# Ipsedo/MARLClassification

Measured on NVIDIA B200. Metric: image_episodes_per_sec, higher is better.
Workload: dtype tf32x3

## Files before the change

marlclassification_b200/csrc/engine.cu:

```cuda
#include <stdarg.h>
#include <string.h>

#include <algorithm>

#include <string>
#include <vector>

#include <nvtx3/nvToolsExt.h>

#include "../../include/marlc.h"
#include "kernels.cuh"
#include "chain.cuh"
#include "tc.cuh"

namespace marlc {

int g_launch_count = 0;
long g_simt_gemm_launches = 0, g_tc_gemm_launches = 0;
static thread_local char g_err[512] = "";
void set_error(const char* fmt, ...) {
    va_list ap;
    va_start(ap, fmt);
    vsnprintf(g_err, sizeof(g_err), fmt, ap);
    va_end(ap);
}
thread_local int g_pdl = 0, g_pdl_trig = 0;
bool pdl_enabled() {
    static const bool on = !(getenv("MARLC_PDL") && atoi(getenv("MARLC_PDL")) == 0);
    return on;
}
int pdl_edge(int bit) {
    static const int mask = getenv("MARLC_PDL_MASK") ? atoi(getenv("MARLC_PDL_MASK")) : 125;
    return (mask & bit) ? 1 : 0;
}
int pdl_trig_mode(int bwd) {
    static const int t = getenv("MARLC_PDL_TRIG") ? atoi(getenv("MARLC_PDL_TRIG")) : 1;
    return (t >> (bwd ? 1 : 0)) & 1;
}
int pdl_trigger_early() { return g_pdl_trig; }

struct ParamInfo {
    std::string name;
    int64_t offset;
    int ndim;
    int64_t shape[4];
    int64_t numel;
};
struct BufInfo {
    std::string name;
    size_t offset, bytes;
};

}

using namespace marlc;

struct NvtxRange {
    explicit NvtxRange(const char* name) { nvtxRangePushA(name); }
    ~NvtxRange() { nvtxRangePop(); }
};

struct marlc_engine {
    marlc_config cfg;
    int M, TM, F, Kin, L;
    CnnDesc cnn;
    int cnn_sz[MAX_CNN_LAYERS];
    std::vector<ParamInfo> params;
    int64_t param_floats = 0;
    std::vector<BufInfo> bufs;
    size_t ws_bytes = 0;
    char* ws = nullptr;
    float* P = nullptr;
    float* G = nullptr;
    int last_launches = 0;
    int debug_stop = 0;
    cudaStream_t side[2] = {nullptr, nullptr};
    cudaStream_t hp = nullptr;
    int bwd_chunks = 1;
    cudaEvent_t ev[64];
    int n_ev = 0, ev_i = 0;
    cudaEvent_t next_event() { cudaEvent_t x = ev[ev_i]; ev_i = (ev_i + 1) % n_ev; return x; }
    int chain(cudaStream_t from, cudaStream_t to) {
        cudaEvent_t x = next_event();
        MARLC_CUDA(cudaEventRecord(x, from));
        MARLC_CUDA(cudaStreamWaitEvent(to, x, 0));
        return 0;
    }

    void add_param(const std::string& name, std::initializer_list<int64_t> shape) {
        ParamInfo p;
        p.name = "_ModelsWrapper__" + name;
        p.ndim = (int)shape.size();
        p.numel = 1;
        int i = 0;
        for (int k = 0; k < 4; ++k) p.shape[k] = 1;
        for (auto s : shape) { p.shape[i++] = s; p.numel *= s; }
        p.offset = param_floats;
        param_floats += (p.numel + 63) / 64 * 64;
        params.push_back(p);
    }
    void add_buf(const std::string& name, size_t bytes) {
        BufInfo b{name, ws_bytes, bytes};
        ws_bytes += (bytes + 255) / 256 * 256;
        bufs.push_back(b);
    }
    const ParamInfo* find_param(const std::string& suffix) const {
        for (auto& p : params)
            if (p.name == "_ModelsWrapper__" + suffix) return &p;
        return nullptr;
    }
    float* prm(const std::string& suffix) const { return P + find_param(suffix)->offset; }
    bool lo_on = false;
    bool h_lo_ok = false;
    const float* lo_of(const float* p) const {
        if (!lo_on || !p) return nullptr;
        struct R { const float* base; size_t n; const float* lo; };
        const size_t Ms = (size_t)M, T1 = (size_t)cfg.T + 1;
        const R r[] = {{P, (size_t)param_floats, buf("params_lo")},
                       {buf("H"), T1 * Ms * cfg.n_b, buf("H_lo")},
                       {buf("Hc"), T1 * Ms * cfg.n_a, buf("Hc_lo")}
                       };
        for (int i = 0; i < 3; ++i) {
            const R& q = r[i];
            if (i > 0 && !h_lo_ok) break;
            if (q.lo && p >= q.base && p < q.base + q.n) return q.lo + (p - q.base);
        }
        return nullptr;
    }
    TcOperand op(const float* p, long ld, bool mn = false) const {
        TcOperand o = tc_op(p, ld, mn);
        o.lo = lo_of(p);
        return o;
    }
    float* grd(const std::string& suffix) const { return G + find_param(suffix)->offset; }
    template <typename T = float>
    T* buf(const std::string& name) const {
        for (auto& b : bufs)
            if (b.name == name) return reinterpret_cast<T*>(ws + b.offset);
        return nullptr;
    }
};

static const char* CNN_PREFIX = "map_obs._Generic2dCnnModule__layers.";
static const char* LSTM_B = "belief_unit._LSTMCellWrapper__lstm.";
static const char* LSTM_A = "action_unit._LSTMCellWrapper__lstm.";

static void add_block(marlc_engine* e, const std::string& name, int i, int n_in, int n_out, bool norm) {
    e->add_param(name + "." + std::to_string(i) + ".weight", {n_out, n_in});
    e->add_param(name + "." + std::to_string(i) + ".bias", {n_out});
    if (norm) {
        e->add_param(name + "." + std::to_string(i + 1) + ".weight", {n_out});
        e->add_param(name + "." + std::to_string(i + 1) + ".bias", {n_out});
    }
}

extern "C" int marlc_version(void) { return 1; }

extern "C" long marlc_selftest_fastdiv(int d_max, int stride) {
    long bad = 0;
    if (stride < 1) stride = 1;
    for (int d = 1; d <= d_max; ++d) {
// ... 75 lines not shown

    const size_t M = e->M, TM = e->TM, T = c->T, F4 = sizeof(float);
    e->add_buf("rng_state", 2 * sizeof(uint64_t));
    e->add_buf("pos_hist", (T + 1) * M * 2 * sizeof(int));
    e->add_buf("npos", (T + 1) * M * 2 * F4);
    e->add_buf("act", TM * sizeof(int));
    e->add_buf("zero_act", M * sizeof(int64_t));
    e->add_buf("step_pos", TM * 2 * sizeof(int64_t));
    for (int l = 0; l < e->L; ++l) e->add_buf("cnn_y" + std::to_string(l), TM * e->cnn_sz[l] * F4);
    e->add_buf("U", TM * e->Kin * F4);
    e->add_buf("msg", (T + 1) * M * c->n_m * F4);
    e->add_buf("coll", TM * c->n_m * F4);
    e->add_buf("dec_y1", TM * 2 * c->n_m * F4);
    e->add_buf("dec_s1", TM * 2 * c->n_m * F4);
    e->add_buf("dec_y2", TM * c->n_m_o * F4);
    e->add_buf("pos_y", TM * c->n_d * F4);
    e->add_buf("H", (T + 1) * M * c->n_b * F4);
    e->add_buf("Cb", (T + 1) * M * c->n_b * F4);
    e->add_buf("Hc", (T + 1) * M * c->n_a * F4);
    e->add_buf("Cc", (T + 1) * M * c->n_a * F4);
    e->add_buf("gates_b", TM * 4 * c->n_b * F4);
    e->add_buf("gates_a", TM * 4 * c->n_a * F4);
    e->add_buf("enc_y1", TM * 2 * c->n_m * F4);
    e->add_buf("enc_s1", TM * 2 * c->n_m * F4);
    e->add_buf("enc_y2", TM * c->n_m * F4);
    e->add_buf("pol_y1", TM * c->nl_a * F4);
    e->add_buf("pol_s1", TM * c->nl_a * F4);
    e->add_buf("probs", TM * c->n_actions * F4);
    e->add_buf("cri_y1", TM * c->nl_a * F4);
    e->add_buf("cri_s1", TM * c->nl_a * F4);
    e->add_buf("prd_y1", TM * c->nl_b * F4);
    e->add_buf("prd_s1", TM * c->nl_b * F4);
    e->add_buf("step_preds", TM * c->nb_class * F4);
    e->add_buf("step_log_probas", TM * F4);
    e->add_buf("step_values", TM * F4);
    e->add_buf("rewards", TM * F4);
    e->add_buf("returns", TM * F4);
    e->add_buf("adv", TM * F4);
    e->add_buf("loss_stats", 16 * sizeof(double));
    e->add_buf("loss_out", 8 * F4);
    e->add_buf("d_preds", TM * c->nb_class * F4);
    e->add_buf("d_logp", TM * F4);
    e->add_buf("d_values", TM * F4);
    const size_t nl_max = (size_t)std::max(c->nl_a, c->nl_b);
    e->add_buf("d_pol_logits", TM * c->n_actions * F4);
    e->add_buf("scratchS", TM * nl_max * F4);
    e->add_buf("scratchY", TM * nl_max * F4);
    e->add_buf("scratchS2", TM * nl_max * F4);
    e->add_buf("scratchY2", TM * nl_max * F4);
    e->add_buf("scratchS3", TM * nl_max * F4);
    e->add_buf("scratchY3", TM * nl_max * F4);
    e->add_buf("dH_heads", TM * c->n_b * F4);
    e->add_buf("dHc_heads", TM * c->n_a * F4);
    e->add_buf("dgates_b", TM * 4 * c->n_b * F4);
    e->add_buf("dgates_a", TM * 4 * c->n_a * F4);
    e->add_buf("dU", TM * e->Kin * F4);
    e->add_buf("d_enc_y2", TM * c->n_m * F4);
    e->add_buf("d_enc_y1", TM * 2 * c->n_m * F4);
    e->add_buf("d_dec_y2", TM * c->n_m_o * F4);
    e->add_buf("d_dec_y1", TM * 2 * c->n_m * F4);
    e->add_buf("d_pos_y", TM * c->n_d * F4);
    e->add_buf("tmpS", M * 2 * c->n_m * F4);
    e->add_buf("dcoll", M * c->n_m * F4);
    e->add_buf("dmsg", M * c->n_m * F4);
    e->add_buf("dh_hist", TM * c->n_b * F4);
    e->add_buf("dhc_hist", TM * c->n_a * F4);
    e->add_buf("dh", M * c->n_b * F4);
    e->add_buf("dc0", M * c->n_b * F4);
    e->add_buf("dc1", M * c->n_b * F4);
    e->add_buf("dhc", M * c->n_a * F4);
    e->add_buf("dcc0", M * c->n_a * F4);
    e->add_buf("dcc1", M * c->n_a * F4);
    if (e->cfg.use_chains)
        for (int l = 0; l < e->L; ++l)
            e->add_buf("cnn_wT" + std::to_string(l), (size_t)d.cout[l] * d.cin[l] * 9 * F4);
    if (e->lo_on) {
        e->add_buf("params_lo", (size_t)e->param_floats * F4);
        e->add_buf("U_lo", M * e->Kin * F4);
        e->add_buf("H_lo", (T + 1) * M * c->n_b * F4);
        e->add_buf("Hc_lo", (T + 1) * M * c->n_a * F4);
        e->add_buf("dgates_b_lo", M * 4 * c->n_b * F4);
        e->add_buf("dgates_a_lo", M * 4 * c->n_a * F4);
    }
    for (int l = 0; l < e->L; ++l) {
        const size_t npos = (size_t)d.hout[l] * d.hout[l];
        e->add_buf("cnn_dY" + std::to_string(l), TM * npos * d.cout[l] * F4);
        e->add_buf("cnn_col" + std::to_string(l), TM * npos * (size_t)((d.cin[l] * 9 + 3) & ~3) * F4);
        e->add_buf("cnn_gnpart" + std::to_string(l), TM * 2 * d.cout[l] * F4);
        if (l > 0) e->add_buf("cnn_dcol" + std::to_string(l), TM * npos * d.cin[l] * 9 * F4);
    }
    *out = e;
    return 0;
}

extern "C" void marlc_engine_destroy(marlc_engine* e) {
    if (!e) return;
    for (int i = 0; i < e->n_ev; ++i) cudaEventDestroy(e->ev[i]);
    for (int i = 0; i < 2; ++i)
        if (e->side[i]) cudaStreamDestroy(e->side[i]);
    if (e->hp) cudaStreamDestroy(e->hp);
    delete e;
}
extern "C" int marlc_engine_param_count(const marlc_engine* e) { return (int)e->params.size(); }
extern "C" int64_t marlc_engine_param_floats(const marlc_engine* e) { return e->param_floats; }
extern "C" int marlc_engine_param_info(const marlc_engine* e, int idx, char* name, int64_t* offset, int* ndim,
                                       int64_t* shape) {
    MARLC_CHECK(idx >= 0 && idx < (int)e->params.size(), "param index %d out of range", idx);
    const ParamInfo& p = e->params[idx];
    strncpy(name, p.name.c_str(), 127);
    name[127] = 0;
    *offset = p.offset;
    *ndim = p.ndim;
    for (int k = 0; k < 4; ++k) shape[k] = p.shape[k];
    return 0;
}
extern "C" size_t marlc_engine_workspace_bytes(const marlc_engine* e) { return e->ws_bytes; }
extern "C" int marlc_engine_buffer(const marlc_engine* e, const char* name, size_t* offset, size_t* nbytes) {
    for (auto& b : e->bufs)
        if (b.name == name) {
            *offset = b.offset;
            *nbytes = b.bytes;
            return 0;
        }
    MARLC_FAIL("unknown workspace buffer '%s'", name);
}

extern "C" int marlc_engine_bind(marlc_engine* e, void* workspace, float* params, float* grads) {
    MARLC_CHECK(workspace && params, "bind: null workspace / params");
    MARLC_CHECK(((uintptr_t)workspace & 255) == 0 && ((uintptr_t)params & 255) == 0, "bind: buffers must be 256-byte aligned");
    e->ws = (char*)workspace;
    e->P = params;
    e->G = grads;
    if (e->n_ev == 0) {
        for (int i = 0; i < 2; ++i) MARLC_CUDA(cudaStreamCreateWithFlags(&e->side[i], cudaStreamNonBlocking));
        int least = 0, greatest = 0;
        MARLC_CUDA(cudaDeviceGetStreamPriorityRange(&least, &greatest));
        MARLC_CUDA(cudaStreamCreateWithPriority(&e->hp, cudaStreamNonBlocking, greatest));
        if (const char* env = getenv("MARLC_BWD_CHUNKS")) e->bwd_chunks = std::max(1, atoi(env));
        for (int i = 0; i < 64; ++i) {
            MARLC_CUDA(cudaEventCreateWithFlags(&e->ev[i], cudaEventDisableTiming));
            e->n_ev = i + 1;
        }
    }
    for (int l = 0; l < e->L; ++l) {
        e->cnn.w[l] = e->prm(CNN_PREFIX + std::to_string(3 * l) + ".weight");
        e->cnn.b[l] = e->prm(CNN_PREFIX + std::to_string(3 * l) + ".bias");
        e->cnn.gn_w[l] = e->prm(CNN_PREFIX + std::to_string(3 * l + 1) + ".weight");
        e->cnn.gn_b[l] = e->prm(CNN_PREFIX + std::to_string(3 * l + 1) + ".bias");
        e->cnn.wT[l] = e->cfg.use_chains ? e->buf("cnn_wT" + std::to_string(l)) : nullptr;
    }
    return 0;
}

__global__ void seed_kernel(uint64_t* st, uint64_t seed) { st[0] = seed; st[1] = 0; }
extern "C" int marlc_engine_seed(marlc_engine* e, uint64_t seed, void* stream) {
    MARLC_CHECK(e->ws, "engine not bound");
    seed_kernel<<<1, 1, 0, (cudaStream_t)stream>>>(e->buf<uint64_t>("rng_state"), seed);
    MARLC_LAUNCH_CHECK();
    return 0;
}


static inline TcOperand tc_op_lo(const float* p, const float* lo, long ld) {
    TcOperand o = tc_op(p, ld);
    o.lo = lo;
    return o;
}
struct SplitLoArgs { const float* src[3]; float* dst[3]; long n[3]; };
__global__ void __launch_bounds__(256) split_lo_kernel(const SplitLoArgs a) {
    const int k = blockIdx.y;
    const long n4 = a.n[k] >> 2;
    const float4* s4 = reinterpret_cast<const float4*>(a.src[k]);
// ... 491 lines not shown
            TcGemmArgs a;
            a.A = tc_op(Yp, c.nl_a); a.B = e->op(e->prm("policy.0.weight"), c.n_a, true); a.K = c.nl_a;
            a.A2 = tc_op(Yc, c.nl_a); a.B2 = e->op(e->prm("critic.0.weight"), c.n_a, true); a.K2 = c.nl_a;
            a.C = e->buf("dHc_heads"); a.ldc = c.n_a; a.M = TM; a.N = c.n_a; a.x3 = x3_of(e); a.allow_split = 1;
            if (tc_operand_ok(a.A) && tc_operand_ok(a.B) && tc_operand_ok(a.A2) && tc_operand_ok(a.B2)) {
                MARLC_TRY(tc_gemm(a, s));
                dual = true;
            }
        }
        if (!dual) {
            MARLC_TRY(G_nn(e, Yp, c.nl_a, e->prm("policy.0.weight"), c.n_a, e->buf("dHc_heads"), c.n_a, TM, c.nl_a, c.n_a, 0, s));
            MARLC_TRY(G_nn(e, Yc, c.nl_a, e->prm("critic.0.weight"), c.n_a, e->buf("dHc_heads"), c.n_a, TM, c.nl_a, c.n_a, 1, s));
        }
        MARLC_TRY(e->chain(sp, s));
        MARLC_TRY(head_bwd_params(e, "predict", e->buf("d_preds"), c.nb_class, e->buf("prd_s1"), Yq,
                                  H + (size_t)M * c.n_b, c.n_b, c.nl_b, sp));
        MARLC_TRY(e->chain(s, sc));
        MARLC_TRY(head_bwd_params(e, "policy", e->buf("d_pol_logits"), c.n_actions, e->buf("pol_s1"), Yp,
                                  Hc + (size_t)M * c.n_a, c.n_a, c.nl_a, sc));
        MARLC_TRY(head_bwd_params(e, "critic", e->buf("d_values"), 1, e->buf("cri_s1"), Yc, Hc + (size_t)M * c.n_a,
                                  c.n_a, c.nl_a, sc));
    } else {
        MARLC_TRY(head_bwd(e, "predict", e->buf("d_preds"), c.nb_class, e->buf("prd_s1"), e->buf("prd_y1"),
                           H + (size_t)M * c.n_b, c.n_b, c.nl_b, e->buf("dH_heads"), 0, s, 1));
        MARLC_TRY(policy_logit_grad(e->buf("d_logp"), e->buf("probs"), e->buf<int>("act"), e->buf("d_pol_logits"), TM,
                                    c.n_actions, s));
        MARLC_TRY(head_bwd(e, "policy", e->buf("d_pol_logits"), c.n_actions, e->buf("pol_s1"), e->buf("pol_y1"),
                           Hc + (size_t)M * c.n_a, c.n_a, c.nl_a, e->buf("dHc_heads"), 0, s));
        MARLC_TRY(head_bwd(e, "critic", e->buf("d_values"), 1, e->buf("cri_s1"), e->buf("cri_y1"), Hc + (size_t)M * c.n_a,
                           c.n_a, c.nl_a, e->buf("dHc_heads"), 1, s));
    }

    }
    auto join_sides = [&]() -> int {
        if (!c.use_chains) return 0;
        MARLC_TRY(e->chain(e->side[0], s));
        MARLC_TRY(e->chain(e->side[1], s));
        return 0;
    };
    if (e->debug_stop == 1) { MARLC_TRY(join_sides()); e->last_launches = g_launch_count - start; return 0; }
    const bool par = c.use_chains != 0;
    auto batched = [&](int t0, int t1, cudaStream_t sL, cudaStream_t s1, cudaStream_t s0) -> int {
        NvtxRange nvtx_batched("marlc/backward/batched_grads");
        const size_t r0 = (size_t)t0 * M;
        const int R = (t1 - t0) * M;
        if (R <= 0) return 0;
        {
            const float* dgb = e->buf("dgates_b") + r0 * 4 * c.n_b;
            const float* dga = e->buf("dgates_a") + r0 * 4 * c.n_a;
            const float* Ur = e->buf("U") + r0 * Kin;
            const std::string pb = LSTM_B, pa = LSTM_A;
            const TnProblem ih[2] = {{dgb, 4L * c.n_b, Ur, Kin, e->grd(pb + "weight_ih"), Kin, R, 4 * c.n_b, Kin},
                                     {dga, 4L * c.n_a, Ur, Kin, e->grd(pa + "weight_ih"), Kin, R, 4 * c.n_a, Kin}};
            const TnProblem hh[2] = {{dgb, 4L * c.n_b, H + r0 * c.n_b, c.n_b, e->grd(pb + "weight_hh"), c.n_b, R, 4 * c.n_b, c.n_b},
                                     {dga, 4L * c.n_a, Hc + r0 * c.n_a, c.n_a, e->grd(pa + "weight_hh"), c.n_a, R, 4 * c.n_a, c.n_a}};
            MARLC_TRY(G_tn_group(e, ih, 2, sL));
            MARLC_TRY(G_tn_group(e, hh, 2, sL));
            MARLC_TRY(colsum_add2(dgb, 4 * c.n_b, e->grd(pb + "bias_ih"), e->grd(pb + "bias_hh"), R, 4 * c.n_b, sL));
            MARLC_TRY(colsum_add2(dga, 4 * c.n_a, e->grd(pa + "bias_ih"), e->grd(pa + "bias_hh"), R, 4 * c.n_a, sL));
        }
        {
            const int Re = (std::min(t1, T - 1) - t0) * M;
            const TnProblem enc[2] = {
                {e->buf("d_enc_y2") + r0 * c.n_m, c.n_m, e->buf("enc_s1") + r0 * 2 * c.n_m, 2L * c.n_m,
                 e->grd("encode_msg.3.weight"), 2L * c.n_m, Re, c.n_m, 2 * c.n_m},
                {e->buf("d_enc_y1") + r0 * 2 * c.n_m, 2L * c.n_m, H + (r0 + M) * c.n_b, c.n_b,
                 e->grd("encode_msg.0.weight"), c.n_b, Re, 2 * c.n_m, c.n_b}};
            if (Re > 0) MARLC_TRY(G_tn_group(e, enc, 2, s1));
            const TnProblem dec[2] = {
                {e->buf("d_dec_y2") + r0 * c.n_m_o, c.n_m_o, e->buf("dec_s1") + r0 * 2 * c.n_m, 2L * c.n_m,
                 e->grd("decode_msg.3.weight"), 2L * c.n_m, R, c.n_m_o, 2 * c.n_m},
                {e->buf("d_dec_y1") + r0 * 2 * c.n_m, 2L * c.n_m, e->buf("coll") + r0 * c.n_m, c.n_m,
                 e->grd("decode_msg.0.weight"), c.n_m, R, 2 * c.n_m, c.n_m}};
            MARLC_TRY(G_tn_group(e, dec, 2, s1));
        }
        MARLC_TRY(block_bwd_norm(e, "map_pos", 0, dU + r0 * Kin + F + c.n_m_o, Kin, e->buf("pos_y") + r0 * c.n_d, R, c.n_d,
                                 e->buf("d_pos_y") + r0 * c.n_d, s1));
        MARLC_TRY(G_tn(e, e->buf("d_pos_y") + r0 * c.n_d, c.n_d, e->buf("npos") + r0 * 2, 2, e->grd("map_pos.0.weight"), 2,
                       R, c.n_d, 2, s1));
        const CnnDesc& d = e->cnn;
        const float* ysave[MAX_CNN_LAYERS];
        CnnBwdBuffers bb;
        float* dcol[MAX_CNN_LAYERS] = {nullptr};
        for (int l = 0; l < e->L; ++l) {
            const size_t npos = (size_t)d.hout[l] * d.hout[l];
            ysave[l] = e->buf("cnn_y" + std::to_string(l)) + (par ? r0 * e->cnn_sz[l] : 0);
            bb.dY[l] = e->buf("cnn_dY" + std::to_string(l)) + (par ? r0 * npos * d.cout[l] : 0);
            bb.col[l] = e->buf("cnn_col" + std::to_string(l)) + (par ? r0 * npos * (size_t)((d.cin[l] * 9 + 3) & ~3) : 0);
            bb.gnpart[l] = e->buf("cnn_gnpart" + std::to_string(l)) + (par ? r0 * 2 * d.cout[l] : 0);
            if (l > 0) dcol[l] = e->buf("cnn_dcol" + std::to_string(l)) + (par ? r0 * npos * d.cin[l] * 9 : 0);
        }
        auto conv_weight_grad = [&](int l, cudaStream_t st) -> int {
            const int npos = d.hout[l] * d.hout[l], kk = d.cin[l] * 9, co = d.cout[l];
            const int pitch = (par && l == 0) ? (kk + 3) & ~3 : kk;
            return G_tn(e, bb.dY[l], co, bb.col[l], pitch, e->grd(CNN_PREFIX + std::to_string(3 * l) + ".weight"), kk,
                        R * npos, co, kk, st);
        };
        if (!par) {
            MARLC_TRY(cnn_bwd(e->cnn, img, e->buf<int>("pos_hist"), c.nb, c.H, c.W, M, 0, TM, ysave, dU, Kin, bb, s0));
            for (int l = 0; l < e->L; ++l) {
                const int npos = d.hout[l] * d.hout[l], co = d.cout[l];
                const std::string cw = CNN_PREFIX + std::to_string(3 * l), gn = CNN_PREFIX + std::to_string(3 * l + 1);
                MARLC_TRY(conv_weight_grad(l, s0));
                MARLC_TRY(colsum_add(bb.dY[l], co, e->grd(cw + ".bias"), R * npos, co, s0));
                MARLC_TRY(colsum_add(bb.gnpart[l], 2 * co, e->grd(gn + ".weight"), R, co, s0));
                MARLC_TRY(colsum_add(bb.gnpart[l] + co, 2 * co, e->grd(gn + ".bias"), R, co, s0));
            }
            return 0;
        }
        MARLC_TRY(cnn_im2col_input(img, e->buf<int>("pos_hist") + r0 * 2, bb.col[0], R, M, c.nb, c.C, d.cin[0], c.H, c.W,
                                   c.f, d.hout[0], s1));
        for (int l = e->L - 1; l >= 0; --l) {
            CnnBwdLayerArgs la;
            memset(&la, 0, sizeof(la));
            la.cout = d.cout[l]; la.ho = d.hout[l]; la.groups = d.groups[l]; la.P = R;
            la.Y = ysave[l]; la.gn_w = d.gn_w[l]; la.gn_b = d.gn_b[l];
            const bool top = (l == e->L - 1);
            la.dOut = top ? dU + r0 * Kin : nullptr; la.lddo = Kin;
            la.dColNext = top ? nullptr : dcol[l + 1];
            la.ho_next = top ? 1 : d.hout[l + 1];
            la.dY = bb.dY[l]; la.gnpart = nullptr;
            la.d_gn_w = e->grd(CNN_PREFIX + std::to_string(3 * l + 1) + ".weight");
            la.d_gn_b = e->grd(CNN_PREFIX + std::to_string(3 * l + 1) + ".bias");
            la.d_conv_b = e->grd(CNN_PREFIX + std::to_string(3 * l) + ".bias");
            la.colNext = top ? nullptr : bb.col[l + 1];
            MARLC_TRY(cnn_bwd_layer(la, s0));
            if (l > 0) {
                const int npos = d.hout[l] * d.hout[l], kk = d.cin[l] * 9;
                MARLC_TRY(G_nn_on(e, bb.dY[l], d.cout[l], d.w[l], kk, dcol[l], kk, R * npos, d.cout[l], kk, s0));
            }
        }
        {
            cudaStream_t fan[3] = {s0, s1, sL};
            cudaEvent_t done = e->next_event();
            MARLC_CUDA(cudaEventRecord(done, s0));
            if (s1 != s0) MARLC_CUDA(cudaStreamWaitEvent(s1, done, 0));
            if (sL != s0) MARLC_CUDA(cudaStreamWaitEvent(sL, done, 0));
            for (int l = e->L - 1, i = 0; l >= 0; --l, ++i) MARLC_TRY(conv_weight_grad(l, l == 0 ? s1 : fan[(i & 1) ? 2 : 0]));
        }
        return 0;
    };
    NvtxRange nvtx_sweep("marlc/backward/sweep");
    float* dh = e->buf("dh");
    float* dhc = e->buf("dhc");
    float* dc[2] = {e->buf("dc0"), e->buf("dc1")};
    float* dcc[2] = {e->buf("dcc0"), e->buf("dcc1")};
    float* dmsg = e->buf("dmsg");
    float* tmpS = e->buf("tmpS");
    MARLC_CUDA(cudaMemsetAsync(dh, 0, sizeof(float) * (size_t)M * c.n_b, s));
    MARLC_CUDA(cudaMemsetAsync(dhc, 0, sizeof(float) * (size_t)M * c.n_a, s));
    MARLC_CUDA(cudaMemsetAsync(dc[0], 0, sizeof(float) * (size_t)M * c.n_b, s));
    MARLC_CUDA(cudaMemsetAsync(dcc[0], 0, sizeof(float) * (size_t)M * c.n_a, s));
    int cur = 0;
    static const int unfused_min_m = getenv("MARLC_SWEEP_UNFUSED_MIN_M") ? atoi(getenv("MARLC_SWEEP_UNFUSED_MIN_M")) : 4096;
    const bool chain_sweep = c.use_chains && M < unfused_min_m;
    if (chain_sweep) {
        float* dcoll = e->buf("dcoll");
        float* dh_hist = e->buf("dh_hist");
        float* dhc_hist = e->buf("dhc_hist");
        MARLC_CUDA(cudaMemsetAsync(dU, 0, sizeof(float) * (size_t)TM * Kin, s));
        MARLC_CUDA(cudaMemsetAsync(dh_hist, 0, sizeof(float) * (size_t)TM * c.n_b, s));
        MARLC_CUDA(cudaMemsetAsync(dhc_hist, 0, sizeof(float) * (size_t)TM * c.n_a, s));
        const bool profiling_stop = e->debug_stop == 2 || e->debug_stop == 21 || e->debug_stop == 22;
        const int nch = profiling_stop ? 0 : std::max(1, std::min(e->bwd_chunks, T));
        cudaStream_t sw = e->hp, s0 = e->side[0], s1 = e->side[1];
        MARLC_TRY(e->chain(s, sw));
        int chunk_hi = T, next_chunk = nch - 1;
        for (int t = T - 1; t >= 0; --t) {
            float* dgb = e->buf("dgates_b") + (size_t)t * M * 4 * c.n_b;
            float* dga = e->buf("dgates_a") + (size_t)t * M * 4 * c.n_a;
            float* dgb_lo = e->lo_on ? e->buf("dgates_b_lo") : nullptr;
            float* dga_lo = e->lo_on ? e->buf("dgates_a_lo") : nullptr;
            BwdPreArgs bp;
            memset(&bp, 0, sizeof(bp));
            bp.dcoll = (t < T - 1) ? dcoll : nullptr;
            bp.e0 = chain_lin(e, "encode_msg", 0, c.n_b, 2 * c.n_m, true);
            bp.e3 = chain_lin(e, "encode_msg", 3, 2 * c.n_m, c.n_m, true);
            bp.enc_y1 = e->buf("enc_y1") + (size_t)t * M * 2 * c.n_m;
            bp.enc_y2 = e->buf("enc_y2") + (size_t)t * M * c.n_m;
            bp.d_enc_y1 = e->buf("d_enc_y1") + (size_t)t * M * 2 * c.n_m;
            bp.d_enc_y2 = e->buf("d_enc_y2") + (size_t)t * M * c.n_m;
            bp.dh_carry[0] = (t < T - 1) ? dh_hist + (size_t)(t + 1) * M * c.n_b : nullptr;
            bp.dh_carry[1] = (t < T - 1) ? dhc_hist + (size_t)(t + 1) * M * c.n_a : nullptr;
            bp.dh_heads[0] = e->buf("dH_heads") + (size_t)t * M * c.n_b;
            bp.dh_heads[1] = e->buf("dHc_heads") + (size_t)t * M * c.n_a;
            bp.dc_next[0] = (t < T - 1) ? dc[cur] : nullptr;
            bp.dc_next[1] = (t < T - 1) ? dcc[cur] : nullptr;
            bp.gates[0] = e->buf("gates_b") + (size_t)t * M * 4 * c.n_b;
            bp.gates[1] = e->buf("gates_a") + (size_t)t * M * 4 * c.n_a;
            bp.c_prev[0] = Cb + (size_t)t * M * c.n_b;
            bp.c_prev[1] = Cc + (size_t)t * M * c.n_a;
            bp.c_new[0] = Cb + (size_t)(t + 1) * M * c.n_b;
            bp.c_new[1] = Cc + (size_t)(t + 1) * M * c.n_a;
            bp.dgates[0] = dgb; bp.dgates[1] = dga;
            bp.dgates_lo[0] = dgb_lo; bp.dgates_lo[1] = dga_lo;
            bp.dc_prev[0] = dc[cur ^ 1]; bp.dc_prev[1] = dcc[cur ^ 1];
            bp.n[0] = c.n_b; bp.n[1] = c.n_a;
            bp.Na = c.na; bp.Nb = c.nb; bp.M = M; bp.n_m = c.n_m;
            {
                PdlScope pdl(t < T - 1 && pdl_edge(PDL_BWD_PRE), pdl_trig_mode(1));
                MARLC_TRY(bwd_pre(bp, sw));
            }
            cur ^= 1;
            if (e->debug_stop == 21) continue;
            float* dUt = dU + (size_t)t * M * Kin;
            float* dh_t = dh_hist + (size_t)t * M * c.n_b;
            float* dhc_t = dhc_hist + (size_t)t * M * c.n_a;
            bool tc_dx = false;
            if (c.use_tc && c.n_a >= 16 && c.n_b >= 16) {
                TcGemmArgs g[3];
                g[0].A = tc_op_lo(dgb, dgb_lo, 4 * c.n_b); g[0].B = e->op(e->prm(std::string(LSTM_B) + "weight_ih"), Kin, true); g[0].K = 4 * c.n_b;
                g[0].A2 = tc_op_lo(dga, dga_lo, 4 * c.n_a); g[0].B2 = e->op(e->prm(std::string(LSTM_A) + "weight_ih"), Kin, true); g[0].K2 = 4 * c.n_a;
                g[0].C = dUt; g[0].ldc = Kin; g[0].M = M; g[0].N = Kin;
// ... 285 lines not shown
```

marlclassification_b200/csrc/kernels.cuh:

```cuda
#pragma once
#include "common.cuh"

namespace marlc {

int patch_gather_i64(const float* img, const int64_t* pos, float* obs, int Na, int B, int C, int H, int W, int f,
                     cudaStream_t s);
int patch_gather_i32(const float* img, const int* pos, float* obs, int Na, int B, int C, int H, int W, int f,
                     cudaStream_t s);
int transition_i64(int64_t* pos, const int64_t* act, const int64_t* table, int nA, int M, int f, int H, int W,
                   float* npos, int* err, cudaStream_t s);
int normalized_positions_i64(const int64_t* pos, float* out, int M, int H, int W, cudaStream_t s);

struct EpisodeInitArgs {
    const int64_t* pos0;
    const float* hidden0[4];
    const uint64_t* rng_state;
    int* pos;
    float* npos;
    float* hidden[4];
    float* msg0;
    int width[4];
    int M, n_m, H, W, f;
};
int episode_init(const EpisodeInitArgs& a, cudaStream_t s);
int rng_advance(uint64_t* rng_state, cudaStream_t s);

struct PolicyActArgs {
    const float* s1;
    const float* W3;
    const float* b3;
    const int64_t* act_in;
    const uint64_t* rng_state;
    const int* pos_in;
    float* probs;
    float* logp;
    int* act_out;
    int* pos_out;
    int64_t* step_pos;
    float* npos_out;
    int moves[32];
    int M, nl, nA, t, f, H, W;
};
int policy_act(const PolicyActArgs& a, cudaStream_t s);

constexpr int MAX_CNN_LAYERS = 6;
struct CnnDesc {
    int L;
    int cin[MAX_CNN_LAYERS], cout[MAX_CNN_LAYERS], groups[MAX_CNN_LAYERS];
    int hin[MAX_CNN_LAYERS], hout[MAX_CNN_LAYERS];
    int f;
    int img_c;
    int out_size;
    const float* w[MAX_CNN_LAYERS];
    const float* b[MAX_CNN_LAYERS];
    const float* gn_w[MAX_CNN_LAYERS];
    const float* gn_b[MAX_CNN_LAYERS];
    const float* wT[MAX_CNN_LAYERS];
};
int cnn_fwd(const CnnDesc& d, const float* img, const int* pos, const float* patch, int B, int H, int W, int M,
            float* const* y_save, float* out, long ldo, cudaStream_t s);

struct CnnBwdBuffers {
    float* dY[MAX_CNN_LAYERS];
    float* col[MAX_CNN_LAYERS];
    float* gnpart[MAX_CNN_LAYERS];
};
int cnn_bwd(const CnnDesc& d, const float* img, const int* pos_hist, int B, int H, int W, int M, int p0, int P,
            const float* const* y_save, const float* dOut, long lddo, const CnnBwdBuffers& buf, cudaStream_t s);

int cnn_weights_transpose(const CnnDesc& d, float* const* wT, cudaStream_t s);

struct CnnBwdLayerArgs {
    int cout, ho, groups;
    int P;
    const float* Y;
    const float* gn_w;
    const float* gn_b;
    const float* dOut;
    long lddo;
    const float* dColNext;
    int ho_next;
    float* dY;
    float* gnpart;
    float* d_gn_w;
    float* d_gn_b;
    float* d_conv_b;
    float* colNext;
};
int cnn_bwd_layer(const CnnBwdLayerArgs& a, cudaStream_t s);
int cnn_im2col_input(const float* img, const int* pos_hist, float* col, int P, int M, int B, int img_c, int cin, int H,
                     int W, int f, int ho, cudaStream_t s);

struct LossArgs {
    const float* preds;
    const float* logp;
    const float* values;
    const int64_t* targets;
    float* rewards;
    float* returns;
    float* adv;
    double* stats;
    float* d_preds;
    float* d_logp;
    float* d_values;
    float* loss_out;
    int T, Na, Nb, Nc;
    float gamma;
};
int loss_phase_a(const LossArgs& a, cudaStream_t s);
int loss_phase_b(const LossArgs& a, cudaStream_t s);
int policy_logit_grad(const float* d_logp, const float* probs, const int* act, float* dlogits, int R, int nA,
                      cudaStream_t s);

}
```

Measured before the change: 19870.

## Fuse backward of first two CNN layers into one persistent kernel

Adds a persistent kernel that fuses, for the first two conv layers, the input-gradient GEMM, col2im, GroupNorm+SiLU backward, and the weight, bias and norm gradient reductions. Per-patch tiles are staged into shared memory with double-buffered cp.async, and gradients are accumulated in registers and flushed with atomics. This removes the im2col/dcol/gnpart workspace buffers and several launches and global round-trips. The trade-off is a fixed-shape specialisation, plain FP32 math instead of tensor cores for these layers, and atomic accumulation that makes gradient sums order-dependent.

```diff
diff --git a/marlclassification_b200/csrc/cnn_bwd_fused.cu b/marlclassification_b200/csrc/cnn_bwd_fused.cu
--- /dev/null
+++ b/marlclassification_b200/csrc/cnn_bwd_fused.cu
@@ -0,0 +1,300 @@
+#include <algorithm>
+
+#include "common.cuh"
+#include "kernels.cuh"
+
+namespace marlc {
+
+namespace {
+constexpr float GN_EPS1 = 1e-5f;
+constexpr int CI = 3, C0 = 16, C1 = 32, H0 = 6, H1 = 3, FW = 12;
+constexpr int N0 = H0 * H0, N1 = H1 * H1, T0 = C0 * N0, K1 = C0 * 9, K0 = CI * 9;
+constexpr int NW = 8;
+constexpr int THREADS = NW * 32;
+constexpr int ACT_LD = N0 + 1;
+constexpr int S_DY1 = N1 * C1;
+constexpr int S_X = T0;
+constexpr int S_IMG = CI * FW * FW;
+constexpr int S_IN = S_DY1 + S_X + S_IMG;
+constexpr int S_DZ = T0;
+constexpr int S_ACT = C0 * ACT_LD;
+constexpr int S_DCOL = N1 * K1;
+constexpr int S_WIN = 2 * S_IN + S_DZ + S_ACT + S_DCOL;
+constexpr int S_TOTAL = C1 * K1 + NW * S_WIN + 3 * C0;
+static_assert(THREADS / 2 == (C1 / 4) * C0, "dW1 ownership: two halves of (4 output x 1 input channel) blocks");
+static_assert(C0 % 4 == 0 && K1 <= 5 * 32 && (S_DY1 % 4) == 0 && (T0 % 4) == 0 && (S_IN % 4) == 0 && (S_WIN % 4) == 0, "layout");
+__device__ __forceinline__ void cp_async16(float* dst, const float* src) {
+    asm volatile("cp.async.cg.shared.global [%0], [%1], 16;" ::"r"((unsigned)__cvta_generic_to_shared(dst)), "l"(src)
+                 : "memory");
+}
+__device__ __forceinline__ void cp_async4(float* dst, const float* src) {
+    asm volatile("cp.async.ca.shared.global [%0], [%1], 4;" ::"r"((unsigned)__cvta_generic_to_shared(dst)), "l"(src)
+                 : "memory");
+}
+}
+
+struct CnnBwdFused10Args {
+    int P, M, B, img_c, H, W;
+    const float* img;
+    const int* pos_hist;
+    const float* dY1;
+    const float* Y0;
+    const float* w1;
+    const float* gn_w0;
+    const float* gn_b0;
+    int groups0;
+    float* dW1;
+    float* dW0;
+    float* d_gn_w0;
+    float* d_gn_b0;
+    float* d_conv_b0;
+};
+
+__global__ void __launch_bounds__(THREADS, 1) cnn_bwd_fused10_kernel(const CnnBwdFused10Args a) {
+    extern __shared__ __align__(16) float sm[];
+    float* sW1 = sm;
+    float* win0 = sm + C1 * K1;
+    float* cta_acc = win0 + NW * S_WIN;
+    const int tid = threadIdx.x, lane = tid & 31, warp = tid >> 5;
+    for (int i = tid; i < C1 * K1 / 4; i += THREADS) reinterpret_cast<float4*>(sW1)[i] = __ldg(reinterpret_cast<const float4*>(a.w1) + i);
+    for (int i = tid; i < 3 * C0; i += THREADS) cta_acc[i] = 0.f;
+
+    float* w_in = win0 + warp * S_WIN;
+    float* w_dz = w_in + 2 * S_IN;
+    float* w_act = w_dz + S_DZ;
+    float* w_dcol = w_act + S_ACT;
+
+    const int h1 = tid >> 7, cq1 = (tid & 127) >> 4, ci1 = tid & 15;
+    const bool own0 = tid < 12 * (N0 / 2);
+    const int cb0 = tid % 12, cq0 = cb0 / 3, ci0 = cb0 % 3, s0 = tid / 12;
+    float acc1[4][9], acc0[4][9];
+#pragma unroll
+    for (int c = 0; c < 4; ++c)
+#pragma unroll
+        for (int k = 0; k < 9; ++k) acc1[c][k] = acc0[c][k] = 0.f;
+    __syncthreads();
+
+    const int G = a.groups0, cpg = C0 / G, ng = cpg * N0;
+    const float inv = 1.0f / (float)ng;
+    const int ntiles = (a.P + NW - 1) / NW;
+    auto issue = [&](int tile, int buf) {
+        if (tile >= ntiles) return;
+        const int p = tile * NW + warp;
+        float* dy1 = w_in + buf * S_IN;
+        float* x = dy1 + S_DY1;
+        float* im = x + S_X;
+        if (p < a.P) {
+            const float* g1 = a.dY1 + (long)p * S_DY1;
+            for (int i = lane; i < S_DY1 / 4; i += 32) cp_async16(dy1 + 4 * i, g1 + 4 * i);
+            const float* g0 = a.Y0 + (long)p * T0;
+            for (int i = lane; i < T0 / 4; i += 32) cp_async16(x + 4 * i, g0 + 4 * i);
+            const int b = (p % a.M) % a.B, py = __ldg(a.pos_hist + 2 * (long)p), px = __ldg(a.pos_hist + 2 * (long)p + 1);
+            const float* src = a.img + ((long)b * a.img_c * a.H + py) * a.W + px;
+            for (int e = lane; e < S_IMG; e += 32) {
+                const int c = e / (FW * FW), r = e - c * FW * FW, y = r / FW, xx = r - y * FW;
+                cp_async4(im + e, src + ((long)c * a.H + y) * a.W + xx);
+            }
+        } else {
+            for (int i = lane; i < S_IN; i += 32) dy1[i] = 0.f;
+        }
+    };
+    issue(blockIdx.x, 0);
+    asm volatile("cp.async.commit_group;" ::: "memory");
+    int cur = 0;
+    for (int tile = blockIdx.x; tile < ntiles; tile += gridDim.x, cur ^= 1) {
+        issue(tile + gridDim.x, cur ^ 1);
+        asm volatile("cp.async.commit_group;" ::: "memory");
+        asm volatile("cp.async.wait_group 1;" ::: "memory");
+        __syncwarp();
+        float* w_dy1 = w_in + cur * S_IN;
+        float* w_x = w_dy1 + S_DY1;
+        {
+            float acc[N1][5];
+#pragma unroll
+            for (int o = 0; o < N1; ++o)
+#pragma unroll
+                for (int q = 0; q < 5; ++q) acc[o][q] = 0.f;
+            const bool q4 = lane + 128 < K1;
+#pragma unroll 4
+            for (int co = 0; co < C1; ++co) {
+                float wv[5];
+#pragma unroll
+                for (int q = 0; q < 4; ++q) wv[q] = sW1[co * K1 + lane + 32 * q];
+                wv[4] = q4 ? sW1[co * K1 + lane + 128] : 0.f;
+#pragma unroll
+                for (int o = 0; o < N1; ++o) {
+                    const float d = w_dy1[o * C1 + co];
+#pragma unroll
+                    for (int q = 0; q < 5; ++q) acc[o][q] = fmaf(d, wv[q], acc[o][q]);
+                }
+            }
+#pragma unroll
+            for (int o = 0; o < N1; ++o) {
+#pragma unroll
+                for (int q = 0; q < 4; ++q) w_dcol[o * K1 + lane + 32 * q] = acc[o][q];
+                if (q4) w_dcol[o * K1 + lane + 128] = acc[o][4];
+            }
+        }
+        __syncwarp();
+        for (int e = lane; e < T0; e += 32) {
+            const int c = e / N0, pos = e - c * N0, iy = pos / H0, ix = pos - iy * H0;
+            float acc = 0.f;
+#pragma unroll
+            for (int ky = 0; ky < 3; ++ky) {
+                const int ty = iy + 1 - ky;
+                if (ty < 0 || (ty & 1) || (ty >> 1) >= H1) continue;
+#pragma unroll
+                for (int kx = 0; kx < 3; ++kx) {
+                    const int tx = ix + 1 - kx;
+                    if (tx < 0 || (tx & 1) || (tx >> 1) >= H1) continue;
+                    acc += w_dcol[((ty >> 1) * H1 + (tx >> 1)) * K1 + c * 9 + ky * 3 + kx];
+                }
+            }
+            w_dz[e] = acc;
+        }
+        __syncwarp();
+        for (int g = 0; g < G; ++g) {
+            float* xg = w_x + g * ng;
+            float* dg = w_dz + g * ng;
+            float s = 0.f;
+            for (int e = lane; e < ng; e += 32) s += xg[e];
+            const float mean = warp_sum(s) * inv;
+            float v = 0.f;
+            for (int e = lane; e < ng; e += 32) { const float d = xg[e] - mean; v += d * d; }
+            const float rstd = 1.0f / sqrtf(warp_sum(v) * inv + GN_EPS1);
+            float s1 = 0.f, s2 = 0.f;
+            for (int e = lane; e < ng; e += 32) {
+                const int cl = e / N0, c = g * cpg + cl;
+                const float gam = __ldg(a.gn_w0 + c);
+                const float x = (xg[e] - mean) * rstd, z = x * gam + __ldg(a.gn_b0 + c);
+                const float sg = sigmoidf_(z);
+                w_act[c * ACT_LD + (e - cl * N0)] = z * sg;
+                const float d = dg[e] * (sg * (1.f + z * (1.f - sg)));
+                xg[e] = x;
+                dg[e] = d;
+                s1 += d * gam;
+                s2 += d * gam * x;
+            }
+            s1 = warp_sum(s1) * inv;
+            s2 = warp_sum(s2) * inv;
+            __syncwarp();
+            for (int cc = lane; cc < cpg; cc += 32) {
+                float t1 = 0.f, t2 = 0.f;
+                for (int q = 0; q < N0; ++q) { const float d = dg[cc * N0 + q]; t1 += d * xg[cc * N0 + q]; t2 += d; }
+                atomicAdd(&cta_acc[g * cpg + cc], t1);
+                atomicAdd(&cta_acc[C0 + g * cpg + cc], t2);
+            }
+            __syncwarp();
+            for (int e = lane; e < ng; e += 32) {
+                const int c = g * cpg + e / N0;
+                dg[e] = rstd * (dg[e] * __ldg(a.gn_w0 + c) - s1 - xg[e] * s2);
+            }
+            __syncwarp();
+            for (int cc = lane; cc < cpg; cc += 32) {
+                float t3 = 0.f;
+                for (int q = 0; q < N0; ++q) t3 += dg[cc * N0 + q];
+                atomicAdd(&cta_acc[2 * C0 + g * cpg + cc], t3);
+            }
+        }
+        __syncthreads();
+#pragma unroll 1
+        for (int w = h1; w < NW; w += 2) {
+            const float* dy = win0 + w * S_WIN + cur * S_IN;
+            const float* act = win0 + w * S_WIN + 2 * S_IN + S_DZ + ci1 * ACT_LD;
+#pragma unroll
+            for (int o = 0; o < N1; ++o) {
+                const int oy = o / H1, ox = o - oy * H1;
+                const float4 d = *reinterpret_cast<const float4*>(dy + o * C1 + 4 * cq1);
+#pragma unroll
+                for (int ky = 0; ky < 3; ++ky) {
+                    const int iy = 2 * oy - 1 + ky;
+#pragma unroll
+                    for (int kx = 0; kx < 3; ++kx) {
+                        const int ix = 2 * ox - 1 + kx;
+                        if (iy < 0 || ix < 0) continue;
+                        const float v = act[iy * H0 + ix];
+                        acc1[0][ky * 3 + kx] = fmaf(d.x, v, acc1[0][ky * 3 + kx]);
+                        acc1[1][ky * 3 + kx] = fmaf(d.y, v, acc1[1][ky * 3 + kx]);
+                        acc1[2][ky * 3 + kx] = fmaf(d.z, v, acc1[2][ky * 3 + kx]);
+                        acc1[3][ky * 3 + kx] = fmaf(d.w, v, acc1[3][ky * 3 + kx]);
+                    }
+                }
+            }
+        }
+        if (own0) {
+#pragma unroll 1
+            for (int w = 0; w < NW; ++w) {
+                const float* dz = win0 + w * S_WIN + 2 * S_IN + 4 * cq0 * N0;
+                const float* im = win0 + w * S_WIN + cur * S_IN + S_DY1 + S_X + ci0 * FW * FW;
+#pragma unroll
+                for (int j = 0; j < 2; ++j) {
+                    const int o = 2 * s0 + j, oy = o / H0, ox = o - oy * H0;
+                    const float d0 = dz[o], d1 = dz[N0 + o], d2 = dz[2 * N0 + o], d3 = dz[3 * N0 + o];
+#pragma unroll
+                    for (int ky = 0; ky < 3; ++ky) {
+                        const int iy = 2 * oy - 1 + ky;
+#pragma unroll
+                        for (int kx = 0; kx < 3; ++kx) {
+                            const int ix = 2 * ox - 1 + kx;
+                            if (iy < 0 || ix < 0) continue;
+                            const float v = im[iy * FW + ix];
+                            acc0[0][ky * 3 + kx] = fmaf(d0, v, acc0[0][ky * 3 + kx]);
+                            acc0[1][ky * 3 + kx] = fmaf(d1, v, acc0[1][ky * 3 + kx]);
+                            acc0[2][ky * 3 + kx] = fmaf(d2, v, acc0[2][ky * 3 + kx]);
+                            acc0[3][ky * 3 + kx] = fmaf(d3, v, acc0[3][ky * 3 + kx]);
+                        }
+                    }
+                }
+            }
+        }
+        __syncthreads();
+    }
+#pragma unroll
+    for (int c = 0; c < 4; ++c)
+#pragma unroll
+        for (int k = 0; k < 9; ++k) atomicAdd(a.dW1 + (4 * cq1 + c) * K1 + ci1 * 9 + k, acc1[c][k]);
+    if (own0) {
+#pragma unroll
+        for (int c = 0; c < 4; ++c)
+#pragma unroll
+            for (int k = 0; k < 9; ++k) atomicAdd(a.dW0 + (4 * cq0 + c) * K0 + ci0 * 9 + k, acc0[c][k]);
+    }
+    for (int i = tid; i < C0; i += THREADS) {
+        atomicAdd(a.d_gn_w0 + i, cta_acc[i]);
+        atomicAdd(a.d_gn_b0 + i, cta_acc[C0 + i]);
+        atomicAdd(a.d_conv_b0 + i, cta_acc[2 * C0 + i]);
+    }
+}
+
+bool cnn_bwd_fused10_supported(const CnnDesc& d) {
+    return d.L >= 2 && d.f == FW && d.cin[0] == CI && d.cout[0] == C0 && d.cout[1] == C1 && d.hout[0] == H0 &&
+           d.hout[1] == H1 && d.groups[0] >= 1 && C0 % d.groups[0] == 0;
+}
+
+int cnn_bwd_fused10(const CnnDesc& d, const float* img, const int* pos_hist, int P, int M, int B, int H, int W,
+                    const float* dY1, const float* Y0, float* dW1, float* dW0, float* d_gn_w0, float* d_gn_b0,
+                    float* d_conv_b0, cudaStream_t s) {
+    if (P <= 0) return 0;
+    MARLC_CHECK(cnn_bwd_fused10_supported(d), "cnn_bwd_fused10: feature extractor shape not supported");
+    MARLC_CHECK(((uintptr_t)dY1 & 15) == 0 && ((uintptr_t)Y0 & 15) == 0 && ((uintptr_t)d.w[1] & 15) == 0,
+                "cnn_bwd_fused10: operands must be 16-byte aligned");
+    CnnBwdFused10Args a;
+    a.P = P; a.M = M; a.B = B; a.img_c = d.img_c; a.H = H; a.W = W;
+    a.img = img; a.pos_hist = pos_hist; a.dY1 = dY1; a.Y0 = Y0; a.w1 = d.w[1];
+    a.gn_w0 = d.gn_w[0]; a.gn_b0 = d.gn_b[0]; a.groups0 = d.groups[0];
+    a.dW1 = dW1; a.dW0 = dW0; a.d_gn_w0 = d_gn_w0; a.d_gn_b0 = d_gn_b0; a.d_conv_b0 = d_conv_b0;
+    const size_t smem = (size_t)S_TOTAL * sizeof(float);
+    static int ctas_per_sm = 0;
+    if (!ctas_per_sm) {
+        MARLC_CUDA(cudaFuncSetAttribute(cnn_bwd_fused10_kernel, cudaFuncAttributeMaxDynamicSharedMemorySize, (int)smem));
+        MARLC_CUDA(cudaOccupancyMaxActiveBlocksPerMultiprocessor(&ctas_per_sm, cnn_bwd_fused10_kernel, THREADS, smem));
+        MARLC_CHECK(ctas_per_sm >= 1, "cnn_bwd_fused10: kernel does not fit an SM");
+    }
+    const int ntiles = (P + NW - 1) / NW;
+    const int grid = std::min(ntiles, 4 * MARLC_SMS * ctas_per_sm);
+    cnn_bwd_fused10_kernel<<<grid, THREADS, smem, s>>>(a);
+    MARLC_LAUNCH_CHECK();
+    return 0;
+}
+
+}
diff --git a/marlclassification_b200/csrc/engine.cu b/marlclassification_b200/csrc/engine.cu
--- a/marlclassification_b200/csrc/engine.cu
+++ b/marlclassification_b200/csrc/engine.cu
@@ -77,6 +77,7 @@
     cudaStream_t side[2] = {nullptr, nullptr};
     cudaStream_t hp = nullptr;
     int bwd_chunks = 1;
+    bool cnn_fused10 = false;
     cudaEvent_t ev[64];
     int n_ev = 0, ev_i = 0;
     cudaEvent_t next_event() { cudaEvent_t x = ev[ev_i]; ev_i = (ev_i + 1) % n_ev; return x; }
@@ -318,12 +319,17 @@
         e->add_buf("dgates_b_lo", M * 4 * c->n_b * F4);
         e->add_buf("dgates_a_lo", M * 4 * c->n_a * F4);
     }
+    {
+        const char* env = getenv("MARLC_CNN_BWD_FUSED");
+        e->cnn_fused10 = e->cfg.use_chains && !(env && atoi(env) == 0) && cnn_bwd_fused10_supported(d);
+    }
     for (int l = 0; l < e->L; ++l) {
         const size_t npos = (size_t)d.hout[l] * d.hout[l];
-        e->add_buf("cnn_dY" + std::to_string(l), TM * npos * d.cout[l] * F4);
-        e->add_buf("cnn_col" + std::to_string(l), TM * npos * (size_t)((d.cin[l] * 9 + 3) & ~3) * F4);
-        e->add_buf("cnn_gnpart" + std::to_string(l), TM * 2 * d.cout[l] * F4);
-        if (l > 0) e->add_buf("cnn_dcol" + std::to_string(l), TM * npos * d.cin[l] * 9 * F4);
+        const bool in_fused = e->cnn_fused10 && l < 2;
+        if (!(in_fused && l == 0)) e->add_buf("cnn_dY" + std::to_string(l), TM * npos * d.cout[l] * F4);
+        if (!in_fused) e->add_buf("cnn_col" + std::to_string(l), TM * npos * (size_t)((d.cin[l] * 9 + 3) & ~3) * F4);
+        if (!e->cnn_fused10) e->add_buf("cnn_gnpart" + std::to_string(l), TM * 2 * d.cout[l] * F4);
+        if (l > 0 && !in_fused) e->add_buf("cnn_dcol" + std::to_string(l), TM * npos * d.cin[l] * 9 * F4);
     }
     *out = e;
     return 0;
@@ -981,13 +987,17 @@
         const float* ysave[MAX_CNN_LAYERS];
         CnnBwdBuffers bb;
         float* dcol[MAX_CNN_LAYERS] = {nullptr};
+        auto ws_at = [&](const std::string& name, size_t off) -> float* {
+            float* p = e->buf(name);
+            return p ? p + (par ? off : 0) : nullptr;
+        };
         for (int l = 0; l < e->L; ++l) {
             const size_t npos = (size_t)d.hout[l] * d.hout[l];
             ysave[l] = e->buf("cnn_y" + std::to_string(l)) + (par ? r0 * e->cnn_sz[l] : 0);
-            bb.dY[l] = e->buf("cnn_dY" + std::to_string(l)) + (par ? r0 * npos * d.cout[l] : 0);
-            bb.col[l] = e->buf("cnn_col" + std::to_string(l)) + (par ? r0 * npos * (size_t)((d.cin[l] * 9 + 3) & ~3) : 0);
-            bb.gnpart[l] = e->buf("cnn_gnpart" + std::to_string(l)) + (par ? r0 * 2 * d.cout[l] : 0);
-            if (l > 0) dcol[l] = e->buf("cnn_dcol" + std::to_string(l)) + (par ? r0 * npos * d.cin[l] * 9 : 0);
+            bb.dY[l] = ws_at("cnn_dY" + std::to_string(l), r0 * npos * d.cout[l]);
+            bb.col[l] = ws_at("cnn_col" + std::to_string(l), r0 * npos * (size_t)((d.cin[l] * 9 + 3) & ~3));
+            bb.gnpart[l] = ws_at("cnn_gnpart" + std::to_string(l), r0 * 2 * d.cout[l]);
+            if (l > 0) dcol[l] = ws_at("cnn_dcol" + std::to_string(l), r0 * npos * d.cin[l] * 9);
         }
         auto conv_weight_grad = [&](int l, cudaStream_t st) -> int {
             const int npos = d.hout[l] * d.hout[l], kk = d.cin[l] * 9, co = d.cout[l];
@@ -1007,9 +1017,12 @@
             }
             return 0;
         }
-        MARLC_TRY(cnn_im2col_input(img, e->buf<int>("pos_hist") + r0 * 2, bb.col[0], R, M, c.nb, c.C, d.cin[0], c.H, c.W,
-                                   c.f, d.hout[0], s1));
-        for (int l = e->L - 1; l >= 0; --l) {
+        const bool fused = e->cnn_fused10;
+        const int lo = fused ? 1 : 0;
+        if (!fused)
+            MARLC_TRY(cnn_im2col_input(img, e->buf<int>("pos_hist") + r0 * 2, bb.col[0], R, M, c.nb, c.C, d.cin[0], c.H,
+                                       c.W, c.f, d.hout[0], s1));
+        for (int l = e->L - 1; l >= lo; --l) {
             CnnBwdLayerArgs la;
             memset(&la, 0, sizeof(la));
             la.cout = d.cout[l]; la.ho = d.hout[l]; la.groups = d.groups[l]; la.P = R;
@@ -1024,10 +1037,22 @@
             la.d_conv_b = e->grd(CNN_PREFIX + std::to_string(3 * l) + ".bias");
             la.colNext = top ? nullptr : bb.col[l + 1];
             MARLC_TRY(cnn_bwd_layer(la, s0));
-            if (l > 0) {
+            if (l > lo) {
                 const int npos = d.hout[l] * d.hout[l], kk = d.cin[l] * 9;
                 MARLC_TRY(G_nn_on(e, bb.dY[l], d.cout[l], d.w[l], kk, dcol[l], kk, R * npos, d.cout[l], kk, s0));
             }
+        }
+        if (fused) {
+            cudaEvent_t done = e->next_event();
+            MARLC_CUDA(cudaEventRecord(done, s0));
+            if (s1 != s0) MARLC_CUDA(cudaStreamWaitEvent(s1, done, 0));
+            if (sL != s0) MARLC_CUDA(cudaStreamWaitEvent(sL, done, 0));
+            for (int l = e->L - 1, i = 0; l >= 2; --l, ++i) MARLC_TRY(conv_weight_grad(l, (i & 1) ? sL : s1));
+            auto grd = [&](int k, const char* what) { return e->grd(CNN_PREFIX + std::to_string(k) + what); };
+            MARLC_TRY(cnn_bwd_fused10(d, img, e->buf<int>("pos_hist") + r0 * 2, R, M, c.nb, c.H, c.W, bb.dY[1], ysave[0],
+                                      grd(3, ".weight"), grd(0, ".weight"), grd(1, ".weight"), grd(1, ".bias"),
+                                      grd(0, ".bias"), s0));
+            return 0;
         }
         {
             cudaStream_t fan[3] = {s0, s1, sL};
diff --git a/marlclassification_b200/csrc/kernels.cuh b/marlclassification_b200/csrc/kernels.cuh
--- a/marlclassification_b200/csrc/kernels.cuh
+++ b/marlclassification_b200/csrc/kernels.cuh
@@ -91,6 +91,11 @@
 int cnn_im2col_input(const float* img, const int* pos_hist, float* col, int P, int M, int B, int img_c, int cin, int H,
                      int W, int f, int ho, cudaStream_t s);
 
+bool cnn_bwd_fused10_supported(const CnnDesc& d);
+int cnn_bwd_fused10(const CnnDesc& d, const float* img, const int* pos_hist, int P, int M, int B, int H, int W,
+                    const float* dY1, const float* Y0, float* dW1, float* dW0, float* d_gn_w0, float* d_gn_b0,
+                    float* d_conv_b0, cudaStream_t s);
+
 struct LossArgs {
     const float* preds;
     const float* logp;
```

After: 20260, median of 6. 1.02x the previous value.
